# yl-jiang/YOLOSeries

Measured on AMD Instinct MI355X. Metric: images/sec (640x640) YOLOv5s train-step, higher is better.
Workload: dtype bf16; 1 GPU; YOLOv5s bf16 train step (fwd+loss+bwd+clip+SGD+EMA), batch 64/GPU x 640x640 synthetic COCO-80, random-init (BASELINE.json configs[1]); global_batch=64, parallelism=dp1

## Files before the change

yoloseries_amd/csrc/conv_wgp.hip:

```cpp
#include "common.h"
#include <stdlib.h>

namespace {

typedef __attribute__((ext_vector_type(4))) short v4s;
typedef __attribute__((ext_vector_type(8))) short v8s;
typedef __attribute__((ext_vector_type(4))) unsigned int u32x4_t;

__device__ __forceinline__ v4s wgp_tr(const uint16_t* p) {
    return __builtin_amdgcn_ds_read_tr16_b64_v4i16((__attribute__((address_space(3))) v4s*)(p));
}

#ifndef WGP_MINB
#define WGP_MINB 3
#endif
constexpr int WGP_TW = 16;

struct WgpK {
    const uint16_t* gy; int ldg, N;
    const uint16_t* x; int ldx, C;
    float* dw; int Ktot, Ctot, coff_k;
    int B, Ho, Wo, Hi, Wi, stride;
    int TH, tx, ty, ntiles, PW, npatch;
    int ntile_n, ntile_c, ntiles_acc, tpw;
    int ntaps, kw_, pad;
    unsigned gybytes, xbytes;
    const uint16_t* z; int ldz; const float* ws; const float* gamma; const float* coef; unsigned zbytes;
};

constexpr int wgp_pitch(int cols) { const int r = (cols + 31) / 32 * 32; return (r % 64 == 32) ? r : r + 32; }

template <int NW, int TPW, int NGI, int NXI, bool FBN>
__device__ __forceinline__ void wgp_body(const WgpK& p, const int PG, const int PX)
{
    constexpr int NT = 64 * NW;
    constexpr unsigned OOB = 0x80000000u;
    extern __shared__ __attribute__((aligned(16))) unsigned char smem[];
    uint16_t* sG = reinterpret_cast<uint16_t*>(smem);
    uint16_t* sX = sG + p.TH * WGP_TW * PG;

    const int t = threadIdx.x;
    const int lane = t & 63;
    const int wave = t >> 6;
    const int s = p.stride;
    const __amdgpu_buffer_rsrc_t rsg = __builtin_amdgcn_make_buffer_rsrc((void*)p.gy, 0, p.gybytes, 0x00020000);
    const __amdgpu_buffer_rsrc_t rsx = __builtin_amdgcn_make_buffer_rsrc((void*)p.x, 0, p.xbytes, 0x00020000);
    const __amdgpu_buffer_rsrc_t rsz = __builtin_amdgcn_make_buffer_rsrc((void*)(FBN ? p.z : p.gy), 0, FBN ? p.zbytes : p.gybytes, 0x00020000);
    float* const sCst = reinterpret_cast<float*>(sX + p.npatch * PX);
    if (FBN) {
        for (int c = t; c < 64; c += NT) {
            const int cc = c < p.N ? c : 0;
            const float mu = p.ws[2 * p.N + cc], is = p.ws[3 * p.N + cc];
            const float gi = p.gamma[cc] * is;
            const float c1 = p.coef[cc], c2 = p.coef[p.N + cc];
            sCst[c] = p.ws[cc]; sCst[64 + c] = p.ws[p.N + cc];
            sCst[128 + c] = gi;
            sCst[192 + c] = -gi * is * c2;
            sCst[256 + c] = gi * (mu * is * c2 - c1);
        }
    }

    const int gch = (p.N + 7) / 8, xch = p.C / 8;
    const int ng_items = p.TH * WGP_TW * gch, nx_items = p.npatch * xch;

    const int g16 = lane >> 4, i16 = lane & 15;
    const int q = i16 >> 2, pp = i16 & 3;
    const int prow = 8 * (g16 >> 1) + q;
    const int chalf = 16 * (g16 & 1) + 4 * pp;

    int a_off[TPW], b_off[TPW];
    bool live[TPW];
#pragma unroll
    for (int k = 0; k < TPW; ++k) {
        const int tile = k * NW + wave;
        live[k] = tile < p.ntiles_acc;
        const int nt = live[k] ? tile / p.ntile_c : 0;
        const int tc = live[k] ? tile - nt * p.ntile_c : 0;
        a_off[k] = prow * PG + nt * 32 + chalf;
        const int col = tc * 32 + chalf;
        const int tap = col / p.C, c = col - tap * p.C;
        const int tp = tap < p.ntaps ? tap : p.ntaps - 1;
        const int kh = tp / p.kw_, kw = tp - kh * p.kw_;
        b_off[k] = (kh * p.PW + kw + prow * s) * PX + c;
    }

    f32x16_t acc[TPW];
#pragma unroll
    for (int k = 0; k < TPW; ++k)
#pragma unroll
        for (int r = 0; r < 16; ++r) acc[k][r] = 0.f;

    u32x4_t rg[NGI], rx[NXI], rz[FBN ? NGI : 1];
    unsigned gok = 0;
    auto tile_origin = [&](int tile, int& b, int& i0, int& j0) {
        const int per = p.tx * p.ty;
        b = tile / per;
        const int r = tile - b * per;
        const int tyi = r / p.tx;
        i0 = tyi * p.TH; j0 = (r - tyi * p.tx) * WGP_TW;
    };
    auto load_regs = [&](int tile) {
        int b, i0, j0;
        tile_origin(tile, b, i0, j0);
#pragma unroll
        for (int j = 0; j < NGI; ++j) {
            const int id = t + j * NT;
            const int px = id / gch, chn = id - px * gch;
            const int i = px / WGP_TW, jj = px - i * WGP_TW;
            const int gi = i0 + i, gj = j0 + jj;
            const bool ok = id < ng_items && gi < p.Ho && gj < p.Wo;
            rg[j] = __builtin_amdgcn_raw_buffer_load_b128(rsg, ok ? (unsigned)(((b * p.Ho + gi) * p.Wo + gj) * (p.ldg * 2) + chn * 16) : OOB, 0, 0);
            if (FBN) {
                rz[j] = __builtin_amdgcn_raw_buffer_load_b128(rsz, ok ? (unsigned)(((b * p.Ho + gi) * p.Wo + gj) * (p.ldz * 2) + chn * 16) : OOB, 0, 0);
                gok = (gok & ~(1u << j)) | ((ok ? 1u : 0u) << j);
            }
        }
        const int pi0 = i0 * s - p.pad, pj0 = j0 * s - p.pad;
#pragma unroll
        for (int j = 0; j < NXI; ++j) {
            const int id = t + j * NT;
            const int px = id / xch, chn = id - px * xch;
            const int pi = px / p.PW, pj = px - pi * p.PW;
            const int gi = pi0 + pi, gj = pj0 + pj;
            const bool ok = id < nx_items && gi >= 0 && gj >= 0 && gi < p.Hi && gj < p.Wi;
            rx[j] = __builtin_amdgcn_raw_buffer_load_b128(rsx, ok ? (unsigned)(((b * p.Hi + gi) * p.Wi + gj) * (p.ldx * 2) + chn * 16) : OOB, 0, 2);
        }
    };
    auto store_regs = [&]() {
#pragma unroll
        for (int j = 0; j < NGI; ++j) {
            const int id = t + j * NT;
            if (id < ng_items) {
                const int px = id / gch, chn = id - px * gch;
                u32x4_t v = rg[j];
                if (FBN) {
                    float g[8], z[8], o[8];
                    unpack8(make_uint4(rg[j].x, rg[j].y, rg[j].z, rg[j].w), g);
                    unpack8(make_uint4(rz[j].x, rz[j].y, rz[j].z, rz[j].w), z);
#pragma unroll
                    for (int e = 0; e < 8; ++e) {
                        const int c = chn * 8 + e;
                        const float a = z[e] * sCst[c] + sCst[64 + c];
                        const float sg = sigmoid_fast(a);
                        const float dz = g[e] * (sg * (1.f + a * (1.f - sg)));
                        o[e] = sCst[128 + c] * dz + (sCst[192 + c] * z[e] + sCst[256 + c]);
                    }
                    const uint4 w = ((gok >> j) & 1u) ? pack8(o) : make_uint4(0, 0, 0, 0);
                    v = u32x4_t{w.x, w.y, w.z, w.w};
                    if (chn * 8 + 8 > p.N) {
                        uint16_t* q = reinterpret_cast<uint16_t*>(&v);
                        for (int e = 0; e < 8; ++e) if (chn * 8 + e >= p.N) q[e] = 0;
                    }
                }
                *reinterpret_cast<u32x4_t*>(sG + px * PG + chn * 8) = v;
            }
        }
#pragma unroll
        for (int j = 0; j < NXI; ++j) {
            const int id = t + j * NT;
            if (id < nx_items) { const int px = id / xch, chn = id - px * xch; *reinterpret_cast<u32x4_t*>(sX + px * PX + chn * 8) = rx[j]; }
        }
    };

    int tile = blockIdx.x;
    if (tile < p.ntiles) load_regs(tile);
    for (; tile < p.ntiles; tile += gridDim.x) {
        __syncthreads();
        store_regs();
        __syncthreads();
        if (tile + (int)gridDim.x < p.ntiles) load_regs(tile + gridDim.x);
        for (int g = 0; g < p.TH; ++g) {
            const uint16_t* ga = sG + g * WGP_TW * PG;
            const uint16_t* xa = sX + g * s * p.PW * PX;
            int last_nt = -1;
            bf16x8_t af = {};
#pragma unroll
            for (int k = 0; k < TPW; ++k) {
                if (!live[k]) continue;
                const int nt = (k * NW + wave) / p.ntile_c;
                if (nt != last_nt) {
                    const v4s lo = wgp_tr(ga + a_off[k]);
                    const v4s hi = wgp_tr(ga + a_off[k] + 4 * PG);
                    const v8s v = {lo[0], lo[1], lo[2], lo[3], hi[0], hi[1], hi[2], hi[3]};
                    af = __builtin_bit_cast(bf16x8_t, v);
                    last_nt = nt;
                }
                const v4s lo = wgp_tr(xa + b_off[k]);
                const v4s hi = wgp_tr(xa + b_off[k] + 4 * s * PX);
                const v8s v = {lo[0], lo[1], lo[2], lo[3], hi[0], hi[1], hi[2], hi[3]};
                acc[k] = __builtin_amdgcn_mfma_f32_32x32x16_bf16(af, __builtin_bit_cast(bf16x8_t, v), acc[k], 0, 0, 0);
            }
        }
    }

#pragma unroll
    for (int k = 0; k < TPW; ++k) {
        if (!live[k]) continue;
        const int tile_id = k * NW + wave;
        const int nt = tile_id / p.ntile_c, tc = tile_id - nt * p.ntile_c;
        const int col = tc * 32 + (lane & 31);
        const int tap = col / p.C, c = col - tap * p.C;
        if (tap >= p.ntaps) continue;
        float* base = p.dw + (size_t)tap * p.Ctot + p.coff_k + c;
#pragma unroll
        for (int r = 0; r < 16; ++r) {
            const int n = nt * 32 + (r & 3) + 8 * (r >> 2) + 4 * (lane >> 5);
            if (n < p.N) atomicAdd(base + (size_t)n * p.Ktot, acc[k][r]);
        }
    }
}

template <int NW, int TPW, int NGI, int NXI>
__global__ __launch_bounds__(64 * NW, (NW >= 8 ? 1 : (TPW <= 2 ? WGP_MINB : 2))) void conv_wgp_kernel(const WgpK p, const int PG, const int PX)
{
    wgp_body<NW, TPW, NGI, NXI, false>(p, PG, PX);
}
template <int NW, int TPW, int NGI, int NXI>
__global__ __launch_bounds__(64 * NW, (NW >= 8 ? 1 : (TPW <= 2 ? WGP_MINB : 2))) void conv_wgpf_kernel(const WgpK p, const int PG, const int PX)
{
    wgp_body<NW, TPW, NGI, NXI, true>(p, PG, PX);
}

struct WgpPlan { WgpK k; int nw, tpw, ngi, nxi, PG, PX, gx, smem; };

bool wgp_plan(const yh_wgrad_desc* d, WgpPlan* pl)
{
    const bool k3 = d->KH == 3 && d->KW == 3 && d->pad == 1 && (d->stride == 1 || d->stride == 2);
    const bool k1 = d->KH == 1 && d->KW == 1 && d->pad == 0 && d->stride == 1;
    if (!(k3 || k1) || d->seg.ups) return false;
    if (d->partial) return false;
    const int C = d->seg.C, N = d->N;
    if (!(C == 16 || C == 32 || C == 64) || N < 8 || N > 64) return false;
    if (d->stride == 2 && C > 32) return false;
    if (d->stride == 2 && (d->Hi != 2 * d->Ho || d->Wi != 2 * d->Wo)) return false;
    if (d->stride == 1 && (d->Hi != d->Ho || d->Wi != d->Wo)) return false;
    const unsigned long gyb = ((unsigned long)d->B * d->Ho * d->Wo - 1) * d->ldg * 2 + (unsigned long)((N + 7) / 8 * 8) * 2;
    const unsigned long xb = ((unsigned long)d->B * d->Hi * d->Wi - 1) * d->seg.ld * 2 + (unsigned long)C * 2;
    if (gyb >= (1ul << 31) || xb >= (1ul << 31)) return false;
    WgpK& k = pl->k;
    const int s = d->stride;
    k.TH = s == 1 ? 16 : 8;
    if (k.TH > d->Ho) k.TH = d->Ho;
    k.ntaps = k3 ? 9 : 1; k.kw_ = k3 ? 3 : 1; k.pad = d->pad;
    k.PW = WGP_TW * s + 2 * d->pad;
    k.npatch = (k.TH * s + 2 * d->pad) * k.PW;
    k.tx = (d->Wo + WGP_TW - 1) / WGP_TW; k.ty = (d->Ho + k.TH - 1) / k.TH;
    k.ntiles = d->B * k.tx * k.ty;
    k.ntile_n = (N + 31) / 32;
    k.ntile_c = (k.ntaps * C + 31) / 32;
    k.ntiles_acc = k.ntile_n * k.ntile_c;
    const int na = k.ntiles_acc;
    const int nw = (na == 5 || na == 10) ? 5 : (na > 20 ? 8 : 4);
    if (d->bn_z && nw != 5) return false;
    pl->nw = nw;
    k.tpw = (na + nw - 1) / nw;
    if (k.tpw > 5) return false;
    pl->tpw = k.tpw;
    const int nt = 64 * nw;
    pl->ngi = (k.TH * WGP_TW * ((N + 7) / 8) + nt - 1) / nt;
    pl->nxi = (k.npatch * (C / 8) + nt - 1) / nt;
    k.gy = d->gy; k.ldg = d->ldg; k.N = N;
    k.x = d->seg.ptr; k.ldx = d->seg.ld; k.C = C;
    k.dw = d->dw; k.Ktot = k.ntaps * d->Ctot; k.Ctot = d->Ctot; k.coff_k = d->coff_k;
    k.B = d->B; k.Ho = d->Ho; k.Wo = d->Wo; k.Hi = d->Hi; k.Wi = d->Wi; k.stride = s;
    k.gybytes = (unsigned)gyb; k.xbytes = (unsigned)xb;
    k.z = d->bn_z; k.ldz = d->bn_ldz; k.ws = d->bn_ws; k.gamma = d->bn_gamma; k.coef = d->bn_coef; k.zbytes = 0;
    if (d->bn_z) {
        if (!d->bn_ws || !d->bn_gamma || !d->bn_coef || d->bn_ldz % 8 || (((uintptr_t)d->bn_z) & 15)) return false;
        const unsigned long zb = ((unsigned long)d->B * d->Ho * d->Wo - 1) * d->bn_ldz * 2 + (unsigned long)((N + 7) / 8 * 8) * 2;
        if (zb >= (1ul << 31)) return false;
        k.zbytes = (unsigned)zb;
    }
    pl->PG = wgp_pitch(k.ntile_n * 32);
    pl->PX = wgp_pitch(C < 32 ? 32 : C);
    pl->smem = (k.TH * WGP_TW * pl->PG + k.npatch * pl->PX) * 2 + (d->bn_z ? 5 * 64 * 4 : 0);
    int occ = (150 * 1024) / pl->smem;
    const int occ_max = nw >= 8 ? 1 : (k.tpw <= 2 ? WGP_MINB : 2);
    if (occ > occ_max) occ = occ_max;
    if (occ < 1) return false;
    int gx = 256 * occ;
    if (d->splits > 0 && d->splits < gx) gx = d->splits;
    pl->gx = k.ntiles < gx ? k.ntiles : gx;
    return true;
}

}

static const int kWgpInst[7][4] = {{5, 1, 4, 3}, {5, 2, 7, 3}, {4, 1, 8, 8}, {4, 3, 4, 6}, {4, 5, 4, 10}, {4, 5, 8, 11}, {8, 5, 4, 6}};
static int wgp_pick(const WgpPlan& pl)
{
    for (int i = 0; i < 7; ++i)
        if (pl.nw == kWgpInst[i][0] && pl.tpw <= kWgpInst[i][1] && pl.ngi <= kWgpInst[i][2] && pl.nxi <= kWgpInst[i][3]) return i;
    return -1;
}
int yh_wgp_ok(const yh_wgrad_desc* d) { WgpPlan pl; return (wgp_plan(d, &pl) && wgp_pick(pl) >= 0) ? 1 : 0; }

extern "C" int yh_conv_wgrad_patch_name(const yh_wgrad_desc* d, char* buf, int buflen)
{
    WgpPlan pl;
    if (!buf || buflen < 40) return YH_EINVAL;
    buf[0] = 0;
    if (!d || !wgp_plan(d, &pl)) return YH_OK;
    const int i = wgp_pick(pl);
    if (i >= 0) snprintf(buf, buflen, "conv_wgp%s_kernel<%d, %d, %d, %d>", d->bn_z ? "f" : "", kWgpInst[i][0], kWgpInst[i][1], kWgpInst[i][2], kWgpInst[i][3]);
    return YH_OK;
}

int yh_wgp_run(const yh_wgrad_desc* d, yh_stream stream)
{
    WgpPlan pl;
    YH_CHECK_ARG(wgp_plan(d, &pl), "yh_conv_wgrad: the patch form (tile_k 40) is not eligible for this layer");
    hipStream_t st = (hipStream_t)stream;
    const int inst = wgp_pick(pl);
    YH_CHECK_ARG(inst >= 0, "yh_conv_wgrad: no patch-form instantiation for this layer");
#define YH_TRY_WGP(I_, NW_, TPW_, NGI_, NXI_)                                                                     \
    if (inst == I_) {                                                                                             \
        static YhDevOnce attr_set;                                                                                   \
        if (attr_set.need()) { attr_set.set((const void*)conv_wgp_kernel<NW_, TPW_, NGI_, NXI_>, hipFuncAttributeMaxDynamicSharedMemorySize, 150 * 1024); attr_set.done();  } \
        conv_wgp_kernel<NW_, TPW_, NGI_, NXI_><<<dim3(pl.gx), dim3(64 * NW_), pl.smem, st>>>(pl.k, pl.PG, pl.PX);  \
    }
#define YH_TRY_WGPF(I_, NW_, TPW_, NGI_, NXI_)                                                                    \
    if (inst == I_ && d->bn_z) {                                                                                  \
        static YhDevOnce attr_set;                                                                                   \
        if (attr_set.need()) { attr_set.set((const void*)conv_wgpf_kernel<NW_, TPW_, NGI_, NXI_>, hipFuncAttributeMaxDynamicSharedMemorySize, 150 * 1024); attr_set.done();  } \
        conv_wgpf_kernel<NW_, TPW_, NGI_, NXI_><<<dim3(pl.gx), dim3(64 * NW_), pl.smem, st>>>(pl.k, pl.PG, pl.PX); \
        YH_CHECK_LAUNCH("yh_conv_wgrad(patch, fused BatchNorm backward)");                                        \
        return YH_OK;                                                                                             \
    }
    YH_TRY_WGPF(0, 5, 1, 4, 3)
    YH_TRY_WGPF(1, 5, 2, 7, 3)
#undef YH_TRY_WGPF
    YH_CHECK_ARG(!d->bn_z, "yh_conv_wgrad: the patch form fuses the BatchNorm backward for the stem shapes only");
    YH_TRY_WGP(0, 5, 1, 4, 3)
    YH_TRY_WGP(1, 5, 2, 7, 3)
    YH_TRY_WGP(2, 4, 1, 8, 8)
    YH_TRY_WGP(3, 4, 3, 4, 6)
    YH_TRY_WGP(4, 4, 5, 4, 10)
    YH_TRY_WGP(5, 4, 5, 8, 11)
    YH_TRY_WGP(6, 8, 5, 4, 6)
#undef YH_TRY_WGP
    YH_CHECK_LAUNCH("yh_conv_wgrad(patch)");
    return YH_OK;
}
```

Before: 5529 images/sec.

## Specialize fused BN-backward patch wgrad kernel for stem geometry

Splits the fused BatchNorm-backward weight-gradient path out of the generic patch kernel into a dedicated body. The new body hardcodes the stem geometry (16 channels, 3x3, stride 1, five waves) as compile-time constants. It precomputes per-thread load offsets and packed staging words, walks tiles incrementally instead of dividing, reads BN constants as float4, and software-pipelines the LDS fragment reads ahead of the MFMAs. Launch bounds are raised for higher occupancy and tile height is set by macros. The cost is a narrow specialization guarded by a runtime geometry check, plus higher register pressure.

```diff
diff --git a/yoloseries_amd/csrc/conv_wgp.hip b/yoloseries_amd/csrc/conv_wgp.hip
--- a/yoloseries_amd/csrc/conv_wgp.hip
+++ b/yoloseries_amd/csrc/conv_wgp.hip
@@ -30,7 +30,7 @@
 
 constexpr int wgp_pitch(int cols) { const int r = (cols + 31) / 32 * 32; return (r % 64 == 32) ? r : r + 32; }
 
-template <int NW, int TPW, int NGI, int NXI, bool FBN>
+template <int NW, int TPW, int NGI, int NXI>
 __device__ __forceinline__ void wgp_body(const WgpK& p, const int PG, const int PX)
 {
     constexpr int NT = 64 * NW;
@@ -45,20 +45,6 @@
     const int s = p.stride;
     const __amdgpu_buffer_rsrc_t rsg = __builtin_amdgcn_make_buffer_rsrc((void*)p.gy, 0, p.gybytes, 0x00020000);
     const __amdgpu_buffer_rsrc_t rsx = __builtin_amdgcn_make_buffer_rsrc((void*)p.x, 0, p.xbytes, 0x00020000);
-    const __amdgpu_buffer_rsrc_t rsz = __builtin_amdgcn_make_buffer_rsrc((void*)(FBN ? p.z : p.gy), 0, FBN ? p.zbytes : p.gybytes, 0x00020000);
-    float* const sCst = reinterpret_cast<float*>(sX + p.npatch * PX);
-    if (FBN) {
-        for (int c = t; c < 64; c += NT) {
-            const int cc = c < p.N ? c : 0;
-            const float mu = p.ws[2 * p.N + cc], is = p.ws[3 * p.N + cc];
-            const float gi = p.gamma[cc] * is;
-            const float c1 = p.coef[cc], c2 = p.coef[p.N + cc];
-            sCst[c] = p.ws[cc]; sCst[64 + c] = p.ws[p.N + cc];
-            sCst[128 + c] = gi;
-            sCst[192 + c] = -gi * is * c2;
-            sCst[256 + c] = gi * (mu * is * c2 - c1);
-        }
-    }
 
     const int gch = (p.N + 7) / 8, xch = p.C / 8;
     const int ng_items = p.TH * WGP_TW * gch, nx_items = p.npatch * xch;
@@ -90,8 +76,7 @@
 #pragma unroll
         for (int r = 0; r < 16; ++r) acc[k][r] = 0.f;
 
-    u32x4_t rg[NGI], rx[NXI], rz[FBN ? NGI : 1];
-    unsigned gok = 0;
+    u32x4_t rg[NGI], rx[NXI];
     auto tile_origin = [&](int tile, int& b, int& i0, int& j0) {
         const int per = p.tx * p.ty;
         b = tile / per;
@@ -110,10 +95,6 @@
             const int gi = i0 + i, gj = j0 + jj;
             const bool ok = id < ng_items && gi < p.Ho && gj < p.Wo;
             rg[j] = __builtin_amdgcn_raw_buffer_load_b128(rsg, ok ? (unsigned)(((b * p.Ho + gi) * p.Wo + gj) * (p.ldg * 2) + chn * 16) : OOB, 0, 0);
-            if (FBN) {
-                rz[j] = __builtin_amdgcn_raw_buffer_load_b128(rsz, ok ? (unsigned)(((b * p.Ho + gi) * p.Wo + gj) * (p.ldz * 2) + chn * 16) : OOB, 0, 0);
-                gok = (gok & ~(1u << j)) | ((ok ? 1u : 0u) << j);
-            }
         }
         const int pi0 = i0 * s - p.pad, pj0 = j0 * s - p.pad;
 #pragma unroll
@@ -132,27 +113,7 @@
             const int id = t + j * NT;
             if (id < ng_items) {
                 const int px = id / gch, chn = id - px * gch;
-                u32x4_t v = rg[j];
-                if (FBN) {
-                    float g[8], z[8], o[8];
-                    unpack8(make_uint4(rg[j].x, rg[j].y, rg[j].z, rg[j].w), g);
-                    unpack8(make_uint4(rz[j].x, rz[j].y, rz[j].z, rz[j].w), z);
-#pragma unroll
-                    for (int e = 0; e < 8; ++e) {
-                        const int c = chn * 8 + e;
-                        const float a = z[e] * sCst[c] + sCst[64 + c];
-                        const float sg = sigmoid_fast(a);
-                        const float dz = g[e] * (sg * (1.f + a * (1.f - sg)));
-                        o[e] = sCst[128 + c] * dz + (sCst[192 + c] * z[e] + sCst[256 + c]);
-                    }
-                    const uint4 w = ((gok >> j) & 1u) ? pack8(o) : make_uint4(0, 0, 0, 0);
-                    v = u32x4_t{w.x, w.y, w.z, w.w};
-                    if (chn * 8 + 8 > p.N) {
-                        uint16_t* q = reinterpret_cast<uint16_t*>(&v);
-                        for (int e = 0; e < 8; ++e) if (chn * 8 + e >= p.N) q[e] = 0;
-                    }
-                }
-                *reinterpret_cast<u32x4_t*>(sG + px * PG + chn * 8) = v;
+                *reinterpret_cast<u32x4_t*>(sG + px * PG + chn * 8) = rg[j];
             }
         }
 #pragma unroll
@@ -210,17 +171,241 @@
     }
 }
 
+#ifndef WGPF_TH1
+#define WGPF_TH1 16
+#endif
+#ifndef WGPF_UNR
+#define WGPF_UNR 4
+#endif
+#ifndef WGPF_UNR2
+#define WGPF_UNR2 2
+#endif
+constexpr int WGPF_UNROLL = WGPF_UNR, WGPF_UNROLL2 = WGPF_UNR2;
+#ifndef WGPF_TH2
+#define WGPF_TH2 16
+#endif
+
+__device__ __forceinline__ unsigned wgpf_keep(unsigned v) { asm volatile("" : "+v"(v)); return v; }
+
+__device__ __forceinline__ bf16x8_t wgp_frag(const uint16_t* p, const int second)
+{
+    const v4s lo = wgp_tr(p), hi = wgp_tr(p + second);
+    const v8s v = {lo[0], lo[1], lo[2], lo[3], hi[0], hi[1], hi[2], hi[3]};
+    return __builtin_bit_cast(bf16x8_t, v);
+}
+
+template <int TPW, int ROWS>
+__device__ __forceinline__ void wgpf_mma(const uint16_t* ga, const uint16_t* xa, f32x16_t (&acc)[TPW])
+{
+    constexpr int PG = wgp_pitch(32 * TPW), PX = wgp_pitch(32), PW = WGP_TW + 2;
+    constexpr int n = ROWS, UNR = TPW == 1 ? WGPF_UNROLL : WGPF_UNROLL2;
+    bf16x8_t a[TPW], b, an[TPW], bn;
+#pragma unroll
+    for (int k = 0; k < TPW; ++k) a[k] = wgp_frag(ga + k * 32, 4 * PG);
+    b = wgp_frag(xa, 4 * PX);
+#pragma unroll UNR
+    for (int g = 0; g < n; ++g) {
+        if (g + 1 < n) {
+#pragma unroll
+            for (int k = 0; k < TPW; ++k) an[k] = wgp_frag(ga + (g + 1) * WGP_TW * PG + k * 32, 4 * PG);
+            bn = wgp_frag(xa + (g + 1) * PW * PX, 4 * PX);
+        }
+#pragma unroll
+        for (int k = 0; k < TPW; ++k) acc[k] = __builtin_amdgcn_mfma_f32_32x32x16_bf16(a[k], b, acc[k], 0, 0, 0);
+#pragma unroll
+        for (int k = 0; k < TPW; ++k) a[k] = an[k];
+        b = bn;
+    }
+}
+
+template <int TPW, int NGI, int NXI>
+__device__ __forceinline__ void wgpf_body(const WgpK& p)
+{
+    constexpr int NW = 5, NT = 64 * NW, C = 16, PW = WGP_TW + 2;
+    constexpr int PG = wgp_pitch(32 * TPW), PX = wgp_pitch(32);
+    constexpr int THF = TPW == 1 ? WGPF_TH1 : WGPF_TH2;
+    constexpr unsigned OOB = 0x80000000u;
+    static_assert(THF * WGP_TW * 4 * TPW <= NGI * NT && (THF + 2) * PW * 2 <= NXI * NT, "staging rounds cover the tile and the patch");
+    static_assert(THF < 31 && THF * WGP_TW * PG * 2 <= 65536, "fields of the staging word");
+    extern __shared__ __attribute__((aligned(16))) unsigned char smem[];
+    const int TH = p.TH;
+    uint16_t* const sG = reinterpret_cast<uint16_t*>(smem);
+    uint16_t* const sX = sG + THF * WGP_TW * PG;
+    float* const sCst = reinterpret_cast<float*>(sX + (THF + 2) * PW * PX);
+
+    const int t = threadIdx.x;
+    const int lane = t & 63;
+    const int wave = __builtin_amdgcn_readfirstlane(t >> 6);
+    const __amdgpu_buffer_rsrc_t rsg = __builtin_amdgcn_make_buffer_rsrc((void*)p.gy, 0, p.gybytes, 0x00020000);
+    const __amdgpu_buffer_rsrc_t rsx = __builtin_amdgcn_make_buffer_rsrc((void*)p.x, 0, p.xbytes, 0x00020000);
+    const __amdgpu_buffer_rsrc_t rsz = __builtin_amdgcn_make_buffer_rsrc((void*)p.z, 0, p.zbytes, 0x00020000);
+    if (t < 64) {
+        const int cc = t < p.N ? t : 0;
+        const float mu = p.ws[2 * p.N + cc], is = p.ws[3 * p.N + cc];
+        const float gi = p.gamma[cc] * is;
+        const float c1 = p.coef[cc], c2 = p.coef[p.N + cc];
+        float* const o = sCst + (t >> 3) * 40 + (t & 7);
+        o[0] = p.ws[cc]; o[8] = p.ws[p.N + cc];
+        o[16] = gi;
+        o[24] = -gi * is * c2;
+        o[32] = gi * (mu * is * c2 - c1);
+    }
+
+    const int gch = (p.N + 7) >> 3;
+    const int ldg2 = p.ldg * 2, ldz2 = p.ldz * 2, ldx2 = p.ldx * 2;
+    constexpr bool OFFS = NGI <= 4;
+    int goff[OFFS ? NGI : 1], zoff[OFFS ? NGI : 1], xoff[NXI];
+    unsigned gword[NGI], xword[NXI];
+#pragma unroll
+    for (int j = 0; j < NGI; ++j) {
+        const int id = t + j * NT;
+        const int px = id / gch, chn = id - px * gch;
+        const int i = px >> 4, jj = px & 15;
+        const bool in = i < THF;
+        if (OFFS) {
+            goff[j] = in ? (i * p.Wo + jj) * ldg2 + chn * 16 : 0;
+            zoff[j] = in ? (i * p.Wo + jj) * ldz2 + chn * 16 : 0;
+        }
+        gword[j] = in ? (unsigned)(px * (PG * 2) + chn * 16) | (unsigned)i << 16 | (unsigned)jj << 21 | (unsigned)chn << 25 : 31u << 16;
+    }
+#pragma unroll
+    for (int j = 0; j < NXI; ++j) {
+        const int id = t + j * NT;
+        const int px = id >> 1, chn = id & 1;
+        const int pi = px / PW, pj = px - pi * PW;
+        xoff[j] = (pi * p.Wi + pj) * ldx2 + chn * 16;
+        xword[j] = (unsigned)pi | (unsigned)pj << 8;
+    }
+
+    const int g16 = lane >> 4, i16 = lane & 15;
+    const int q = i16 >> 2, pp = i16 & 3;
+    const int prow = 8 * (g16 >> 1) + q;
+    const int chalf = 16 * (g16 & 1) + 4 * pp;
+    const int tap = 2 * wave + (g16 & 1);
+    const int tp = tap < 9 ? tap : 8;
+    const int kh = tp / 3, kw = tp - kh * 3;
+    const uint16_t* const fa = sG + prow * PG + chalf;
+    const uint16_t* const fb = sX + (kh * PW + kw + prow) * PX + 4 * pp;
+    const int xl = (t >> 1) * PX + (t & 1) * 8;
+
+    f32x16_t acc[TPW];
+#pragma unroll
+    for (int k = 0; k < TPW; ++k)
+#pragma unroll
+        for (int r = 0; r < 16; ++r) acc[k][r] = 0.f;
+
+    const int per = p.tx * p.ty;
+    int rb = blockIdx.x / per, rty = (blockIdx.x - rb * per) / p.tx, rtx = blockIdx.x - rb * per - rty * p.tx;
+    const int db = gridDim.x / per, dty = (gridDim.x - db * per) / p.tx, dtx = gridDim.x - db * per - dty * p.tx;
+
+    u32x4_t rg[NGI], rz[NGI], rx[NXI];
+    unsigned gok = 0;
+    auto load_regs = [&]() {
+        const int i0 = rty * TH, j0 = rtx * WGP_TW;
+        const int gpix = (rb * p.Ho + i0) * p.Wo + j0;
+        const int sg = gpix * ldg2, sz = gpix * ldz2;
+        const int li = min(TH, p.Ho - i0), lj = p.Wo - j0;
+#pragma unroll
+        for (int j = 0; j < NGI; ++j) {
+            const unsigned w = wgpf_keep(gword[j]);
+            const int i = (w >> 16) & 31, jj = (w >> 21) & 15;
+            const bool ok = i < li && jj < lj;
+            const int pix = i * p.Wo + jj, c16 = (w >> 25) * 16;
+            rg[j] = __builtin_amdgcn_raw_buffer_load_b128(rsg, ok ? (unsigned)((OFFS ? goff[j] : pix * ldg2 + c16) + sg) : OOB, 0, 0);
+            rz[j] = __builtin_amdgcn_raw_buffer_load_b128(rsz, ok ? (unsigned)((OFFS ? zoff[j] : pix * ldz2 + c16) + sz) : OOB, 0, 0);
+            gok = (gok & ~(1u << j)) | ((ok ? 1u : 0u) << j);
+        }
+        const int sx = ((rb * p.Hi + i0 - 1) * p.Wi + j0 - 1) * ldx2;
+        const int lo_i = i0 == 0 ? 1 : 0, lo_j = j0 == 0 ? 1 : 0;
+        const int ni = min(TH + 2, p.Hi + 1 - i0) - lo_i, nj = p.Wi + 1 - j0 - lo_j;
+#pragma unroll
+        for (int j = 0; j < NXI; ++j) {
+            const unsigned w = wgpf_keep(xword[j]);
+            const int pi = w & 255, pj = w >> 8;
+            const bool ok = (unsigned)(pi - lo_i) < (unsigned)ni && (unsigned)(pj - lo_j) < (unsigned)nj;
+            rx[j] = __builtin_amdgcn_raw_buffer_load_b128(rsx, ok ? (unsigned)(xoff[j] + sx) : OOB, 0, 2);
+        }
+    };
+    auto store_regs = [&]() {
+#pragma unroll
+        for (int j = 0; j < NXI; ++j)
+            if ((wgpf_keep(xword[j]) & 255) < (unsigned)(THF + 2)) *reinterpret_cast<u32x4_t*>(sX + xl + j * (NT / 2) * PX) = rx[j];
+#pragma unroll
+        for (int j = 0; j < NGI; ++j) {
+            const unsigned gw = wgpf_keep(gword[j]);
+            if (((gw >> 16) & 31) < (unsigned)THF) {
+                const int chn = gw >> 25;
+                const float4* const cst = reinterpret_cast<const float4*>(sCst + chn * 40);
+                float g[8], z[8], o[8];
+                unpack8(make_uint4(rg[j].x, rg[j].y, rg[j].z, rg[j].w), g);
+                unpack8(make_uint4(rz[j].x, rz[j].y, rz[j].z, rz[j].w), z);
+#pragma unroll
+                for (int h = 0; h < 2; ++h) {
+                    const float4 sc4 = cst[h], sh4 = cst[2 + h], a4 = cst[4 + h], b4 = cst[6 + h], d4 = cst[8 + h];
+                    const float sc[4] = {sc4.x, sc4.y, sc4.z, sc4.w}, sh[4] = {sh4.x, sh4.y, sh4.z, sh4.w};
+                    const float A[4] = {a4.x, a4.y, a4.z, a4.w}, Bc[4] = {b4.x, b4.y, b4.z, b4.w}, D[4] = {d4.x, d4.y, d4.z, d4.w};
+#pragma unroll
+                    for (int e = 0; e < 4; ++e) {
+                        const float zz = z[4 * h + e];
+                        const float a = zz * sc[e] + sh[e];
+                        const float sg = sigmoid_fast(a);
+                        const float dz = g[4 * h + e] * (sg * (1.f + a * (1.f - sg)));
+                        o[4 * h + e] = A[e] * dz + (Bc[e] * zz + D[e]);
+                    }
+                }
+                uint4 w = ((gok >> j) & 1u) ? pack8(o) : make_uint4(0, 0, 0, 0);
+                if (p.N & 7) {
+                    const int nv = p.N - chn * 8;
+                    if (nv < 8) {
+                        uint16_t* const qv = reinterpret_cast<uint16_t*>(&w);
+#pragma unroll
+                        for (int e = 0; e < 8; ++e) if (e >= nv) qv[e] = 0;
+                    }
+                }
+                *reinterpret_cast<u32x4_t*>(reinterpret_cast<unsigned char*>(sG) + (gw & 0xffffu)) = u32x4_t{w.x, w.y, w.z, w.w};
+            }
+        }
+    };
+
+    int tile = blockIdx.x;
+    if (tile < p.ntiles) load_regs();
+    for (; tile < p.ntiles; tile += gridDim.x) {
+        __syncthreads();
+        store_regs();
+        __syncthreads();
+        if (tile + (int)gridDim.x < p.ntiles) {
+            rtx += dtx; if (rtx >= p.tx) { rtx -= p.tx; ++rty; }
+            rty += dty; if (rty >= p.ty) { rty -= p.ty; ++rb; }
+            rb += db;
+            load_regs();
+        }
+        wgpf_mma<TPW, THF>(fa, fb, acc);
+    }
+
+    const int col = wave * 32 + (lane & 31);
+    const int etap = col / C, ec = col - etap * C;
+    if (etap >= 9) return;
+    float* const base = p.dw + (size_t)etap * p.Ctot + p.coff_k + ec;
+#pragma unroll
+    for (int k = 0; k < TPW; ++k)
+#pragma unroll
+        for (int r = 0; r < 16; ++r) {
+            const int n = k * 32 + (r & 3) + 8 * (r >> 2) + 4 * (lane >> 5);
+            if (n < p.N) atomicAdd(base + (size_t)n * p.Ktot, acc[k][r]);
+        }
+}
+
 template <int NW, int TPW, int NGI, int NXI>
 __global__ __launch_bounds__(64 * NW, (NW >= 8 ? 1 : (TPW <= 2 ? WGP_MINB : 2))) void conv_wgp_kernel(const WgpK p, const int PG, const int PX)
 {
-    wgp_body<NW, TPW, NGI, NXI, false>(p, PG, PX);
+    wgp_body<NW, TPW, NGI, NXI>(p, PG, PX);
 }
 template <int NW, int TPW, int NGI, int NXI>
-__global__ __launch_bounds__(64 * NW, (NW >= 8 ? 1 : (TPW <= 2 ? WGP_MINB : 2))) void conv_wgpf_kernel(const WgpK p, const int PG, const int PX)
-{
-    wgp_body<NW, TPW, NGI, NXI, true>(p, PG, PX);
-}
-
+__global__ __launch_bounds__(64 * NW, (TPW == 1 ? 4 : 3)) void conv_wgpf_kernel(const WgpK p, const int PG, const int PX)
+{
+    static_assert(NW == 5, "the fused form is the five-wave stem form");
+    wgpf_body<TPW, NGI, NXI>(p);
+}
 struct WgpPlan { WgpK k; int nw, tpw, ngi, nxi, PG, PX, gx, smem; };
 
 bool wgp_plan(const yh_wgrad_desc* d, WgpPlan* pl)
@@ -240,6 +425,7 @@
     WgpK& k = pl->k;
     const int s = d->stride;
     k.TH = s == 1 ? 16 : 8;
+    if (d->bn_z) k.TH = N <= 32 ? WGPF_TH1 : WGPF_TH2;
     if (k.TH > d->Ho) k.TH = d->Ho;
     k.ntaps = k3 ? 9 : 1; k.kw_ = k3 ? 3 : 1; k.pad = d->pad;
     k.PW = WGP_TW * s + 2 * d->pad;
@@ -273,7 +459,11 @@
     }
     pl->PG = wgp_pitch(k.ntile_n * 32);
     pl->PX = wgp_pitch(C < 32 ? 32 : C);
-    pl->smem = (k.TH * WGP_TW * pl->PG + k.npatch * pl->PX) * 2 + (d->bn_z ? 5 * 64 * 4 : 0);
+    pl->smem = (k.TH * WGP_TW * pl->PG + k.npatch * pl->PX) * 2;
+    if (d->bn_z) {
+        const int thf = N <= 32 ? WGPF_TH1 : WGPF_TH2;
+        pl->smem = (thf * WGP_TW * pl->PG + (thf + 2) * k.PW * pl->PX) * 2 + 5 * 64 * 4;
+    }
     int occ = (150 * 1024) / pl->smem;
     const int occ_max = nw >= 8 ? 1 : (k.tpw <= 2 ? WGP_MINB : 2);
     if (occ > occ_max) occ = occ_max;
@@ -321,6 +511,8 @@
     }
 #define YH_TRY_WGPF(I_, NW_, TPW_, NGI_, NXI_)                                                                    \
     if (inst == I_ && d->bn_z) {                                                                                  \
+        YH_CHECK_ARG(pl.k.ntile_n == TPW_ && pl.PG == wgp_pitch(32 * TPW_) && pl.PX == wgp_pitch(32) && pl.k.C == 16 && pl.k.stride == 1 && pl.k.ntaps == 9, \
+                     "yh_conv_wgrad: the fused patch form is compiled for the stem's geometry");                 \
         static YhDevOnce attr_set;                                                                                   \
         if (attr_set.need()) { attr_set.set((const void*)conv_wgpf_kernel<NW_, TPW_, NGI_, NXI_>, hipFuncAttributeMaxDynamicSharedMemorySize, 150 * 1024); attr_set.done();  } \
         conv_wgpf_kernel<NW_, TPW_, NGI_, NXI_><<<dim3(pl.gx), dim3(64 * NW_), pl.smem, st>>>(pl.k, pl.PG, pl.PX); \
```

After: 5553 images/sec, median of 6. About the same (+0.4%).
